# kakaobrain/hqtransformer

Measured on AMD Instinct MI355X. Metric: images/sec (256x256 class-cond sampling), higher is better.
Workload: dtype bf16

## Files before the change

hqtransformer_amd/csrc/engine.hip:

```cpp
#include "../../include/hqt.h"
#include "kernels.h"
#include "fast_kernels.h"
#include "split_kernels.h"
#include "persist.h"

#include <algorithm>
#include <cmath>
#include <cstdarg>
#include <cstdio>
#include <cstring>
#include <map>
#include <memory>
#include <mutex>
#include <string>
#include <vector>

static thread_local std::string g_err;
static int fail(int code, const char* fmt, ...) {
    char buf[1024];
    va_list ap;
    va_start(ap, fmt);
    vsnprintf(buf, sizeof(buf), fmt, ap);
    va_end(ap);
    g_err = buf;
// ... 8 lines not shown
#define CHK(expr)                  \
    do {                           \
        int r_ = (expr);           \
        if (r_ != HQT_OK) return r_; \
    } while (0)

struct DeviceGuard {
    int prev = -1;
    bool ok = false;
    explicit DeviceGuard(int dev) {
        if (hipGetDevice(&prev) != hipSuccess) prev = -1;
        ok = prev == dev || hipSetDevice(dev) == hipSuccess;
        if (prev == dev) prev = -1;
    }
    ~DeviceGuard() { if (prev >= 0) hipSetDevice(prev); }
};
#define ON_DEVICE(h_)                                                                          \
    DeviceGuard dg_((h_)->device);                                                             \
    if (!dg_.ok) return fail(HQT_ERR_HIP, "hipSetDevice(%d) failed", (h_)->device)

struct Tensor {
    float* d = nullptr;
    std::vector<int64_t> shape;
    size_t n = 0;
};

struct Lin {
    const float* w32 = nullptr;
    const float* b32 = nullptr;
    bf16_t* w16 = nullptr;
    half_t* w16h = nullptr;
    half_t* w16l = nullptr;
    float* w32t = nullptr;
    half_t* wfrag16 = nullptr;
    half_t* wup16 = nullptr;
    bf16_t* wpk = nullptr;
    bf16_t* wpk_ln = nullptr;
    float* colsum = nullptr;
    float* bias_ln = nullptr;
    int N = 0, K = 0;
};

struct BlockW {
    bool body = false;
    const float *ln1_g, *ln1_b, *ln2_g, *ln2_b;
    Lin qkv, proj, fc1, fc2;
};

struct DecLayer {
    int kind;
    std::string name;
    int cin, cout, res;
    Lin conv1, conv2, nin, q, k, v, proj;
    const float *n1_g = nullptr, *n1_b = nullptr, *n2_g = nullptr, *n2_b = nullptr;
};

struct PersistProg {
    std::vector<PersistPhase> phases;
    char* stream = nullptr;
    unsigned long long* d_cu_off = nullptr;
    PersistPhase* d_phases = nullptr;
    bool ok = false;
};

struct TimingSlot {
    std::string name;
    std::vector<std::pair<hipEvent_t, hipEvent_t>> ev;
    size_t used = 0;
    int64_t launches = 0;
    double total_ms = 0.0;
};

struct hqt_handle {
    hqt_config cfg;
    int device = 0;
    bool finalized = false;
    std::map<std::string, Tensor> w;
    std::vector<void*> owned;
    size_t workspace_bytes = 0;
    int64_t params[3] = {0, 0, 0};
    std::vector<BlockW> body, depth;
    Lin head_top, head_bot;
    int Tmax = 0;
    int max_prefix = 0;
    static constexpr int BODY_BUFS = 10;
    size_t body_bytes[BODY_BUFS] = {};
    int depth_rows = 0;
    int score_chunk = 0;
    int depth_cap() const { return std::max(cfg.max_batch, score_chunk); }
    static constexpr int DEPTH_BUFS = 4;
    size_t depth_bytes[DEPTH_BUFS] = {};
    float *x = nullptr, *xd = nullptr, *logits = nullptr;
    void *hbuf = nullptr, *qbuf = nullptr, *abuf = nullptr, *mbuf = nullptr;
    void *kcache = nullptr, *vcache = nullptr, *dk = nullptr, *dv = nullptr;
    bf16_t *xpk = nullptr, *xdpk = nullptr;
    float *parts = nullptr, *partsd = nullptr;
    int nparts = 0, npartsd = 0;
    float* fold_tmp = nullptr;
    bool tile_gemm = true;
    float* splitk = nullptr;
    size_t splitk_elems = 0;
    struct { const float* slabs; int S; int rows; const float* bias; } pend = {nullptr, 0, 0, nullptr};
    StepState* state = nullptr;
    RowKey* rows = nullptr;
    static constexpr int ROWS_RING = 4;
    RowKey* rows_pinned[ROWS_RING] = {nullptr, nullptr, nullptr, nullptr};
// ... 573 lines not shown
    CHK(get_w(h, p + ".attn.value.weight", {D, D}, &wv));
    CHK(get_w(h, p + ".attn.query.bias", {D}, &bq));
    CHK(get_w(h, p + ".attn.key.bias", {D}, &bk));
    CHK(get_w(h, p + ".attn.value.bias", {D}, &bv));
    float *wqkv, *bqkv;
    CHK(dev_alloc(h, (void**)&wqkv, (size_t)3 * D * D * 4, false));
    CHK(dev_alloc(h, (void**)&bqkv, (size_t)3 * D * 4, false));
    HIPCHK(hipMemcpy(wqkv, wq, D * D * 4, hipMemcpyDeviceToDevice));
    HIPCHK(hipMemcpy(wqkv + D * D, wk, D * D * 4, hipMemcpyDeviceToDevice));
    HIPCHK(hipMemcpy(wqkv + 2 * D * D, wv, D * D * 4, hipMemcpyDeviceToDevice));
    HIPCHK(hipMemcpy(bqkv, bq, D * 4, hipMemcpyDeviceToDevice));
    HIPCHK(hipMemcpy(bqkv + D, bk, D * 4, hipMemcpyDeviceToDevice));
    HIPCHK(hipMemcpy(bqkv + 2 * D, bv, D * 4, hipMemcpyDeviceToDevice));
    CHK(make_lin(h, b.qkv, wqkv, bqkv, 3 * D, D, true, true));
    CHK(get_w(h, p + ".attn.proj.weight", {D, D}, &w));
    CHK(get_w(h, p + ".attn.proj.bias", {D}, &bias));
    CHK(make_lin(h, b.proj, w, bias, D, D, true, true));
    CHK(get_w(h, p + ".mlp.0.weight", {4 * D, D}, &w));
    CHK(get_w(h, p + ".mlp.0.bias", {4 * D}, &bias));
    CHK(make_lin(h, b.fc1, w, bias, 4 * D, D, true, true));
    CHK(get_w(h, p + ".mlp.2.weight", {D, 4 * D}, &w));
    CHK(get_w(h, p + ".mlp.2.bias", {D}, &bias));
    CHK(make_lin(h, b.fc2, w, bias, D, 4 * D, true, true));
    CHK(fold_ln(h, b.qkv, b.ln1_g, b.ln1_b));
    CHK(fold_ln(h, b.fc1, b.ln2_g, b.ln2_b));
    return HQT_OK;
}

static int load_conv(hqt_handle* h, const std::string& name, int O, int I, int ksz, Lin& l, bool upsampling = false) {
    const float *w, *b;
    CHK(get_w(h, "stage1." + name + ".weight", {O, I, ksz, ksz}, &w));
    CHK(get_w(h, "stage1." + name + ".bias", {O}, &b));
    const int taps = ksz * ksz;
    float* wt = const_cast<float*>(w);
    if (taps > 1) {
        CHK(dev_alloc(h, (void**)&wt, (size_t)O * I * taps * 4, false));
        HIPCHK(launch_repack_conv(w, wt, O, I, taps, 0));
    }
    CHK(make_lin(h, l, wt, b, O, I * taps, false, true));
    if (taps == 9 && I % 32 == 0) {
        if (O % 128 == 0 || O <= 16) {
            CHK(dev_alloc(h, (void**)&l.wfrag16, split_frag_elems(O, I) * sizeof(half_t), false));
            HIPCHK(launch_pack_split_frag16(wt, l.wfrag16, O, I, 0));
        }
        if (upsampling && O % 128 == 0 && I % 64 == 0) {
            CHK(dev_alloc(h, (void**)&l.wup16, split_up_elems(O, I) * sizeof(half_t), false));
            HIPCHK(hipMemset(l.wup16, 0, split_up_elems(O, I) * sizeof(half_t)));
            HIPCHK(launch_pack_split_up16(wt, l.wup16, O, I, 0));
        }
    }
    return HQT_OK;
}

static int conv_in_cpad(const hqt_config& c) { return c.s1_use_init_downsample ? 4 : 16; }

static int load_encoder(hqt_handle* h) {
    const hqt_config& c = h->cfg;
    for (auto& l : h->enc) {
        if (l.kind == 6) {
            const int ks = c.s1_use_init_downsample ? 4 : 3, taps = ks * ks, cp = conv_in_cpad(c);
            const float *w, *b;
            CHK(get_w(h, "stage1.encoder.conv_in.weight", {l.cout, 3, ks, ks}, &w));
            CHK(get_w(h, "stage1.encoder.conv_in.bias", {l.cout}, &b));
            float* wt;
            CHK(dev_alloc(h, (void**)&wt, (size_t)l.cout * cp * taps * 4, false));
            HIPCHK(launch_repack_conv(w, wt, l.cout, 3, taps, 0, cp));
            CHK(make_lin(h, l.conv1, wt, b, l.cout, cp * taps, false));
        } else if (l.kind == 5) {
            CHK(load_conv(h, l.name, l.cout, l.cin, 3, l.conv1));
        } else if (l.kind == 1) {
            CHK(get_w(h, "stage1." + l.name + ".norm1.weight", {l.cin}, &l.n1_g));
            CHK(get_w(h, "stage1." + l.name + ".norm1.bias", {l.cin}, &l.n1_b));
            CHK(get_w(h, "stage1." + l.name + ".norm2.weight", {l.cout}, &l.n2_g));
            CHK(get_w(h, "stage1." + l.name + ".norm2.bias", {l.cout}, &l.n2_b));
            CHK(load_conv(h, l.name + ".conv1", l.cout, l.cin, 3, l.conv1));
            CHK(load_conv(h, l.name + ".conv2", l.cout, l.cout, 3, l.conv2));
            if (l.cin != l.cout) CHK(load_conv(h, l.name + ".nin_shortcut", l.cout, l.cin, 1, l.nin));
        } else if (l.kind == 2) {
            CHK(get_w(h, "stage1." + l.name + ".norm.weight", {l.cin}, &l.n1_g));
            CHK(get_w(h, "stage1." + l.name + ".norm.bias", {l.cin}, &l.n1_b));
            CHK(load_conv(h, l.name + ".q", l.cin, l.cin, 1, l.q));
            CHK(load_conv(h, l.name + ".k", l.cin, l.cin, 1, l.k));
            CHK(load_conv(h, l.name + ".v", l.cin, l.cin, 1, l.v));
            CHK(load_conv(h, l.name + ".proj_out", l.cin, l.cin, 1, l.proj));
        } else {
            CHK(get_w(h, "stage1.encoder.norm_out.weight", {l.cin}, &l.n1_g));
            CHK(get_w(h, "stage1.encoder.norm_out.bias", {l.cin}, &l.n1_b));
            CHK(load_conv(h, "encoder.conv_out", l.cout, l.cin, 3, l.conv1));
        }
    }
    const int E = c.s1_embed_dim, L = c.code_levels == 3 ? 3 : 2;
    CHK(load_conv(h, "quant_conv_b", E, c.s1_z_channels, 1, h->quant_conv));
    if (c.s1_resample == HQT_RESAMPLE_CONV2) {
        const float *w, *b;
        CHK(get_w(h, "stage1.down_t.weight", {E, E, 2, 2}, &w));
        CHK(get_w(h, "stage1.down_t.bias", {E}, &b));
        h->down_lin = Lin();
        h->down_lin.w32 = w; h->down_lin.b32 = b; h->down_lin.N = E; h->down_lin.K = 4 * E;
    }
    for (int l = 0; l < L; ++l) {
        const int dim = c.s1_resample ? E : E << (2 * (L - 1 - l));
        const std::string name = L == 3 ? "stage1.quantizers." + std::to_string(l) + ".embedding"
                                        : (l == 0 ? "stage1.quantize_t.embedding" : "stage1.quantize_b.embedding");
        const float* e = h->w[name].d;
        CHK(dev_alloc(h, (void**)&h->cb_norm[l], (size_t)c.s1_n_embed * 4, false));
        HIPCHK(launch_row_sumsq(e, DT_F32, h->cb_norm[l], c.s1_n_embed, dim, 0));
    }
    h->has_encoder = true;
    return alloc_encode_workspace(h);
}

static std::string key2(const hqt_handle* h, const char* name);

static int finalize_impl(hqt_handle* h);
static int persist_build(hqt_handle* h);
extern "C" int hqt_finalize_weights(hqt_handle* h) {
    if (!h) return fail(HQT_ERR_INVALID, "null handle");
    if (h->finalized) return HQT_OK;
    DeviceGuard dg(h->device);
    if (!dg.ok) return fail(HQT_ERR_HIP, "hipSetDevice(%d) failed", h->device);
    const size_t owned_before = h->owned.size();
    const int rc = finalize_impl(h);
    if (h->fold_tmp) { hipFree(h->fold_tmp); h->fold_tmp = nullptr; }
    if (rc != HQT_OK) {
        hipDeviceSynchronize();
        for (size_t i = owned_before; i < h->owned.size(); ++i) hipFree(h->owned[i]);
        h->owned.resize(owned_before);
        h->body.clear(); h->depth.clear();
        h->pbody = PersistProg(); h->pfull = PersistProg();
        h->head_top = h->head_bot = h->head_l2 = h->post_quant = h->quant_conv = Lin();
        for (auto& l : h->dec) { l.conv1 = l.conv2 = l.nin = l.q = l.k = l.v = l.proj = Lin(); }
        for (auto& l : h->enc) { l.conv1 = l.conv2 = l.nin = l.q = l.k = l.v = l.proj = Lin(); }
        for (auto& p : h->cb_norm) p = nullptr;
        h->vq_h = h->vq_recon = h->vq_zz = h->vq_err = nullptr; h->vq_z = nullptr; h->vq_best = nullptr;
        h->vq_t = h->vq_q = nullptr; h->up_table = nullptr; h->up_lin = h->down_lin = Lin();
        h->has_encoder = false;
    }
// ... 51 lines not shown
            }
            HIPCHK(hipDeviceSynchronize());
        }
        CHK(persist_build(h));
        if (c.cond_type == HQT_COND_CLASS) CHK(get_w(h, "stage2.sos.weight", {c.n_classes, D}, &t));
        else if (c.cond_type == HQT_COND_TEXT) {
            CHK(get_w(h, "stage2.tok_emb_txt.weight", {c.vocab_txt, D}, &t));
            CHK(get_w(h, "stage2.pos_emb_txt.weight", {c.ctx_len_txt, D}, &t));
        } else CHK(get_w(h, "stage2.sos", {1, 1, D}, &t));
    }
    if (c.has_stage1) {
        const int E = c.s1_embed_dim;
        const float* t;
        if (c.code_levels == 3) {
            CHK(get_w(h, "stage1.quantizers.0.embedding", {c.s1_n_embed, 16 * E}, &t));
            CHK(get_w(h, "stage1.quantizers.1.embedding", {c.s1_n_embed, 4 * E}, &t));
            CHK(get_w(h, "stage1.quantizers.2.embedding", {c.s1_n_embed, E}, &t));
            CHK(load_conv(h, "post_quant_conv_b", c.s1_z_channels, E, 1, h->post_quant));
        } else {
            CHK(get_w(h, "stage1.quantize_t.embedding", {c.s1_n_embed, c.s1_resample ? E : 4 * E}, &t));
            if (c.s1_resample == HQT_RESAMPLE_CONV2) {
                const float *uw, *ub;
                CHK(get_w(h, "stage1.upsample_t.weight", {E, E, 2, 2}, &uw));
                CHK(get_w(h, "stage1.upsample_t.bias", {E}, &ub));
                CHK(dev_alloc(h, (void**)&h->up_table, (size_t)c.s1_n_embed * 4 * E * 4, false));
                HIPCHK(launch_fold_upsample_t(t, uw, ub, h->up_table, c.s1_n_embed, E, 0));
                float *wt, *b4;
                CHK(dev_alloc(h, (void**)&wt, (size_t)4 * E * E * 4, false));
                CHK(dev_alloc(h, (void**)&b4, (size_t)4 * E * 4, false));
                HIPCHK(launch_repack_upsample_t(uw, ub, wt, b4, E, 0));
                h->up_lin = Lin();
                h->up_lin.w32 = wt; h->up_lin.b32 = b4; h->up_lin.N = 4 * E; h->up_lin.K = E;
            }
            CHK(get_w(h, "stage1.quantize_b.embedding", {c.s1_n_embed, E}, &t));
            CHK(load_conv(h, "post_quant_conv_b", c.s1_z_channels, 2 * E, 1, h->post_quant));
        }
        for (auto& l : h->dec) {
            if (l.kind == 0 || l.kind == 3) CHK(load_conv(h, l.name, l.cout, l.cin, 3, l.conv1, l.kind == 3));
            else if (l.kind == 1) {
                CHK(get_w(h, "stage1." + l.name + ".norm1.weight", {l.cin}, &l.n1_g));
                CHK(get_w(h, "stage1." + l.name + ".norm1.bias", {l.cin}, &l.n1_b));
                CHK(get_w(h, "stage1." + l.name + ".norm2.weight", {l.cout}, &l.n2_g));
                CHK(get_w(h, "stage1." + l.name + ".norm2.bias", {l.cout}, &l.n2_b));
                CHK(load_conv(h, l.name + ".conv1", l.cout, l.cin, 3, l.conv1));
                CHK(load_conv(h, l.name + ".conv2", l.cout, l.cout, 3, l.conv2));
                if (l.cin != l.cout) CHK(load_conv(h, l.name + ".nin_shortcut", l.cout, l.cin, 1, l.nin));
            } else if (l.kind == 2) {
                CHK(get_w(h, "stage1." + l.name + ".norm.weight", {l.cin}, &l.n1_g));
                CHK(get_w(h, "stage1." + l.name + ".norm.bias", {l.cin}, &l.n1_b));
                CHK(load_conv(h, l.name + ".q", l.cin, l.cin, 1, l.q));
                CHK(load_conv(h, l.name + ".k", l.cin, l.cin, 1, l.k));
                CHK(load_conv(h, l.name + ".v", l.cin, l.cin, 1, l.v));
                CHK(load_conv(h, l.name + ".proj_out", l.cin, l.cin, 1, l.proj));
            } else {
                CHK(get_w(h, "stage1.decoder.norm_out.weight", {l.cin}, &l.n1_g));
                CHK(get_w(h, "stage1.decoder.norm_out.bias", {l.cin}, &l.n1_b));
                CHK(load_conv(h, "decoder.conv_out", l.cout, l.cin, 3, l.conv1));
            }
        }
    }
    if (c.has_stage1 && h->w.count("stage1.encoder.conv_in.weight") && (c.s1_resample != HQT_RESAMPLE_CONV2 || h->w.count("stage1.down_t.weight")))
        CHK(load_encoder(h));
    HIPCHK(stream_gemm_configure());
    HIPCHK(tile_gemm_configure());
    HIPCHK(mfma_gemm_configure());
    HIPCHK(split_kernels_configure());
    HIPCHK(hipDeviceSynchronize());
    h->finalized = true;
    return HQT_OK;
}

struct Mode {
    bool fast = false;
    bool split = false;
    bool split_ar = false;
    int act_dt() const { return fast ? DT_BF16 : DT_F32; }
    size_t act_sz() const { return fast ? 2 : 4; }
};
static int mode_of(int precision, bool stage1, Mode* md) {
    if (precision == HQT_PRECISION_FAST) md->fast = true;
    else if (precision == HQT_PRECISION_SPLIT && stage1) md->split = true;
    else if (precision == HQT_PRECISION_SPLIT) md->split_ar = true;
    else if (precision != HQT_PRECISION_EXACT) return fail(HQT_ERR_INVALID, "unknown precision %d", precision);
    return HQT_OK;
}

static void lin_args(const hqt_handle* h, GemmArgs& g, const Lin& l, bool split_planes) {
    g.N = l.N; g.K = l.K; g.ldb = l.K;
    g.bias = l.b32;
    g.zero_page = h->zero_page;
    g.tune = h->policy;
    if (g.alpha == 0.0f) g.alpha = 1.0f;
    if (g.lda == 0) g.lda = l.K;
    if (split_planes) { g.Bw = l.w16h; g.Bw_lo = l.w16l; g.Bw_frag16 = l.wfrag16; g.Bw_up16 = l.wup16; }
}

struct SlotName {
    char s[64];
    SlotName(const char* tag, int rows) {
        static const bool by_rows = getenv("HQT_TIMING_BY_ROWS") != nullptr;
        snprintf(s, sizeof s, by_rows ? "%s@%d" : "%s", tag, rows);
    }
};

static int ar_linear(hqt_handle* h, const Mode& md, GemmArgs g, const Lin& l, int a_dt, int c_dt, hipStream_t st,
                     const char* tag, bool defer_residual = false, int* resid_nparts = nullptr) {
// ... 1276 lines not shown
    hqt_handle* h = c.h;
    hipStream_t st = c.st;
    const int adt = c.adt, n = c.n;
    void *&cur = c.cur, *&t1 = c.t1, *&t2 = c.t2;
    const int res = l.res, hw = res * res;
    if (l.kind == 0 || l.kind == 3) {
        const int ro = l.kind == 3 ? 2 * res : res;
        GemmArgs g = conv_args(cur, n, ro, l.cin, 9, l.kind == 3, t1, l.cout);
        S1Operand a = S1_PLANES;
        if (c.cur_planes) c.cur_planes = false;
        else CHK(s1_plain(c, &g, l.conv1, &a));
        CHK(s1_conv(c, g, a, l.conv1, adt, "conv3x3"));
        std::swap(cur, t1);
    } else if (l.kind == 5) {
        GemmArgs g = conv_args(cur, n, res / 2, l.cin, 9, 0, t1, l.cout);
        g.conv_stride2 = 1; g.conv_nopad = 1;
        CHK(s1_conv(c, g, S1_TENSOR, l.conv1, adt, "conv_down"));
        std::swap(cur, t1);
    } else if (l.kind == 1) {
        GemmArgs g = conv_args(cur, n, res, l.cin, 9, 0, t1, l.cout);
        S1Operand a;
        CHK(s1_norm(c, cur, l.cin, hw, c.gn1, l.n1_g, l.n1_b, 1, &g, l.conv1, &a));
        CHK(s1_conv(c, g, a, l.conv1, adt, "conv3x3"));
        const void* shortcut = cur;
        void* outbuf = t2;
        if (l.cin != l.cout) {
            GemmArgs sc = conv_args(cur, n, res, l.cin, 1, 0, t2, l.cout);
            CHK(s1_plain(c, &sc, l.nin, &a));
            CHK(s1_conv(c, sc, a, l.nin, adt, "conv1x1"));
            shortcut = t2;
            outbuf = cur;
        }
        g = conv_args(t1, n, res, l.cout, 9, 0, outbuf, l.cout);
        g.resid = shortcut;
        CHK(s1_norm(c, t1, l.cout, hw, c.gn2, l.n2_g, l.n2_b, 1, &g, l.conv2, &a));
        bool planes = false;
        if (a == S1_PLANES && next && next->kind == 3 && next->cin == l.cout) {
            GemmArgs up = conv_args(outbuf, n, 2 * res, next->cin, 9, 1, t1, next->cout);
            GemmArgs me = g;
            lin_args(h, me, l.conv2, true);
            planes = split_shape_ok(h, up, next->conv1) && split_conv3_emits_planes(me);
        }
        if (planes) { g.out_split = 1; g.range_flag = h->range_flag; }
        CHK(s1_conv(c, g, a, l.conv2, adt, "conv3x3"));
        if (outbuf == t2) std::swap(cur, t2);
        c.cur_planes = planes;
        if (planes) count_variant(h, "variant:conv3x3_planes_out:conv3x3");
    } else if (l.kind == 2) {
        const int C = l.cin;
        GemmArgs g = conv_args(cur, n, res, C, 1, 0, h->aq, C);
        S1Operand a;
        CHK(s1_norm(c, cur, C, hw, c.gn1, l.n1_g, l.n1_b, 0, &g, l.q, &a));
        const GemmArgs normed = g;
        CHK(s1_conv(c, g, a, l.q, adt, "conv1x1"));
        g = normed; g.C = h->ak;
        CHK(s1_conv(c, g, a, l.k, adt, "conv1x1"));
        g = normed; g.C = h->av;
        g.store = STORE_NCHW; g.rows_per_image = hw;
        CHK(s1_conv(c, g, a, l.v, adt, "conv1x1"));
        auto product = [&](const void* A, const void* B, void* out, int M, int N, int K, float alpha) -> int {
            Timed t(h, "attn_gemm", st);
            GemmArgs sg{};
            sg.A = A; sg.lda = K; sg.a_batch_stride = (long long)M * K;
            sg.Bw = B; sg.ldb = K; sg.b_batch_stride = (long long)N * K;
            sg.C = out; sg.ldc = N; sg.c_batch_stride = (long long)M * N;
            sg.M = M; sg.N = N; sg.K = K; sg.batch = n; sg.alpha = alpha; sg.store = STORE_ROWS;
            sg.zero_page = h->zero_page;
            if (c.md.fast && mfma_gemm_ok(sg, adt, adt, adt)) {
                count_variant(h, "variant:mfma_gemm:attn_gemm");
                HIPCHK(launch_mfma_gemm(sg, adt, adt, adt, st));
            } else if (s1_split_product(h, c.md, sg)) {
                count_variant(h, "variant:split_gemm:attn_gemm");
                HIPCHK(launch_split_gemm(sg, st));
            } else {
                count_variant(h, c.md.fast ? "variant:gemm_generic_bf16:attn_gemm" : "variant:gemm_generic_f32:attn_gemm");
                HIPCHK(launch_gemm_generic(sg, adt, adt, adt, st));
            }
            return HQT_OK;
        };
        CHK(product(h->aq, h->ak, h->as, hw, hw, C, 1.0f / sqrtf((float)C)));
        { Timed t(h, "softmax", st); HIPCHK(launch_softmax_rows(h->as, adt, n * hw, hw, st)); }
        CHK(product(h->as, h->av, h->ao, hw, C, hw, 1.0f));
        g = conv_args(h->ao, n, res, C, 1, 0, t1, C);
        g.resid = cur;
        CHK(s1_plain(c, &g, l.proj, &a));
        CHK(s1_conv(c, g, a, l.proj, adt, "conv1x1"));
        std::swap(cur, t1);
    } else {
        return fail(HQT_ERR_INVALID, "s1_layer: kind %d", l.kind);
    }
    return HQT_OK;
}

static int decode_chunk(hqt_handle* h, int n, const int64_t* code_t, const int64_t* code_m, const int64_t* code_b, int seq_layout,
                        float* out, int clamp01, const Mode& md, hipStream_t st) {
    const hqt_config& cf = h->cfg;
    const int adt = md.act_dt();
    const int r = h->dec.front().res, E = cf.s1_embed_dim;
    const bool l3 = cf.code_levels == 3;
    {
        Timed t(h, "quant_gather", st);
        if (l3) {
            QuantArgs3 q{code_t, code_m, code_b, seq_layout, W1(h, "quantizers.0.embedding"), W1(h, "quantizers.1.embedding"),
                         W1(h, "quantizers.2.embedding"), h->quant, n, r, E, adt, cf.s1_n_embed};
            HIPCHK(launch_quant_gather3(q, st));
        } else if (cf.s1_resample) {
            const bool conv2 = cf.s1_resample == HQT_RESAMPLE_CONV2;
            QuantRowsArgs q{code_t, code_b, seq_layout, conv2 ? h->up_table : W1(h, "quantize_t.embedding"), conv2 ? 4 : 1,
                            conv2 ? W1(h, "upsample_t.bias") : nullptr, W1(h, "quantize_b.embedding"), h->quant, n, r, E, adt, cf.s1_n_embed};
            HIPCHK(launch_quant_gather_rows(q, st));
        } else {
            QuantArgs q{code_t, code_b, seq_layout, W1(h, "quantize_t.embedding"), W1(h, "quantize_b.embedding"), h->quant, n, r, E, adt, cf.s1_n_embed};
            HIPCHK(launch_quant_gather(q, st));
        }
    }
    S1Ctx c{h, n, md, st, adt, h->act[0], h->act[1], h->act[2], h->act[3], h->gn, h->gn + (size_t)h->dec_chunk * 64};
    {
        GemmArgs g = conv_args(h->quant, n, r, l3 ? E : 2 * E, 1, 0, c.cur, cf.s1_z_channels);
        S1Operand a;
        CHK(s1_plain(c, &g, h->post_quant, &a));
        CHK(s1_conv(c, g, a, h->post_quant, adt, "conv1x1"));
    }
    for (size_t li = 0; li < h->dec.size(); ++li) {
        const DecLayer& l = h->dec[li];
        if (l.kind != 4) { CHK(s1_layer(c, l, li + 1 < h->dec.size() ? &h->dec[li + 1] : nullptr)); continue; }
        const int hw = l.res * l.res;
        GemmArgs g = conv_args(c.cur, n, l.res, l.cin, 9, 0, out, l.cout);
        g.store = STORE_NCHW; g.rows_per_image = hw; g.clamp01 = clamp01;
        if (md.split && l.conv1.w32) {
            GemmArgs d = g;
            d.N = l.conv1.N; d.K = l.conv1.K; d.Bw = l.conv1.w32; d.bias = l.conv1.b32; d.alpha = 1.0f;
            with_gn(d, c.gn1, l.n1_g, l.n1_b, 1);
            if (conv_out_direct_ok(d)) {
                CHK(s1_split_stats(c, c.cur, l.cin, hw, c.gn1));
                Timed t(h, "conv_out", st);
// ... 243 lines not shown
```

hqtransformer_amd/csrc/split_conv.hip:

```cpp
#include "split_kernels.h"
#include "split_ring.h"
#include "gemm_generic.h"
#include <algorithm>
#include <cstdlib>
#include <type_traits>

namespace {
__device__ __forceinline__ unsigned pack_h2(half_t a, half_t b) {
    return (unsigned)__builtin_bit_cast(unsigned short, a) | ((unsigned)__builtin_bit_cast(unsigned short, b) << 16);
}

__device__ __forceinline__ void xcd_tile(int& tile_m, int& tile_n) {
    const int nx = gridDim.x, total = gridDim.x * gridDim.y;
    int id = blockIdx.x + nx * blockIdx.y;
    if ((total & 7) == 0) id = (id & 7) * (total >> 3) + (id >> 3);
    tile_m = id / nx;
    tile_n = id - tile_m * nx;
}
}

__global__ void split_f32_kernel(const float* __restrict__ src, half_t* __restrict__ hi, half_t* __restrict__ lo, size_t n) {
    for (size_t i = blockIdx.x * (size_t)blockDim.x + threadIdx.x; i < n; i += (size_t)gridDim.x * blockDim.x) split2(src[i], hi[i], lo[i]);
}
hipError_t launch_split_f32(const float* src, half_t* hi, half_t* lo, size_t n, hipStream_t st) {
// ... 625 lines not shown
                } else {
#pragma unroll
                    for (int e = 0; e < 4; ++e)
                        if (n4 + e < g.N) {
                            const long long idx = (long long)m * ldc + n4 + e;
                            float x = apply_act(s[e] * g.alpha + bq[e], act);
                            if (Rb) x += Rb[idx];
                            Cb[idx] = x;
                        }
                }
            }
    }
    }
#ifdef HQT_SPLIT_GEMM_STAMPS
    if (g.am_best && tid == 0) {
        st_[3] = clock64();
        long long* d = reinterpret_cast<long long*>(g.am_best) + (size_t)(blockIdx.x + gridDim.x * (blockIdx.y + gridDim.y * blockIdx.z)) * 4;
        d[0] = st_[1] - st_[0]; d[1] = st_[2] - st_[1]; d[2] = st_[3] - st_[2]; d[3] = wall_clock64();
    }
#endif
}

__global__ __launch_bounds__(256) void split_rows_combine_kernel(float* C, int ldc, const float* resid, const float* __restrict__ slabs,
                                                                 const float* __restrict__ bias, int M, int N, int S, int act) {
    const long long i = (long long)blockIdx.x * 256 + threadIdx.x, n4 = N >> 2;
    if (i >= (long long)M * n4) return;
    const int m = (int)(i / n4), n = (int)(i - (long long)m * n4) * 4;
    f32x4 v = *reinterpret_cast<const f32x4*>(slabs + (size_t)m * N + n);
    for (int z = 1; z < S; ++z) v += *reinterpret_cast<const f32x4*>(slabs + ((size_t)z * M + m) * N + n);
    if (bias) v += *reinterpret_cast<const f32x4*>(bias + n);
    if (act != ACT_NONE)
#pragma unroll
        for (int e = 0; e < 4; ++e) v[e] = apply_act(v[e], act);
    if (resid) v += *reinterpret_cast<const f32x4*>(resid + (long long)m * ldc + n);
    *reinterpret_cast<f32x4*>(C + (long long)m * ldc + n) = v;
}

int split_gemm_slices(const GemmArgs& g) {
    if (!g.a_f32 || g.b_f32 || g.store != STORE_ROWS || g.rows_per_group != 0 || g.batch > 1 || g.conv_taps) return 1;
    if (g.N % 4 != 0 || g.ldc % 4 != 0 || g.alpha != 1.0f) return 1;
    const int tiles = ((g.N + 127) / 128) * ((g.M + 127) / 128);
    int S = 1;
    while (S < 4 && g.K % (S * 2 * 64) == 0 && (tiles * S * 2 <= 256 || (tiles * S * 2 <= 512 && g.K / (S * 2) >= 1536))) S *= 2;
    return S;
}

bool split_gemm_ok(const GemmArgs& g) {
    if (!g.zero_page || (!g.Bw_lo && !g.b_f32) || g.gn_stats || g.a_packed_mb || g.a_rows_per_group) return false;
    if (g.conv_taps > 1 || g.conv_stride2 || g.upsample) return false;
    if (g.K % 64 != 0 || g.ldb % 8 != 0) return false;
    if (g.a_f32 && (g.conv_taps ? g.Cin : g.lda) % 4 != 0) return false;
    if (g.b_f32 && (!g.a_f32 || g.ldb % 4 != 0)) return false;
    if (g.store == STORE_QKV)
        return g.a_f32 && !g.b_f32 && g.qkv_D > 0 && g.qkv_D % 64 == 0 && g.N % 64 == 0 && g.ldc % 4 == 0 && g.rows_per_group > 0 && !g.resid && !g.qkv_v_pk && g.batch <= 1;
    if (g.store != STORE_ROWS && g.store != STORE_NCHW) return false;
    if (g.store == STORE_ROWS && g.rows_per_group != 0) return false;
    if (g.store == STORE_NCHW && (g.resid || g.act != ACT_NONE)) return false;
    return true;
}
hipError_t launch_split_gemm(const GemmArgs& g0, hipStream_t st) {
    GemmArgs g = g0;
    if (g.conv_taps == 1) { g.lda = g.a_f32 ? g.Cin : 2 * g.Cin; g.conv_taps = 0; }
    const int a_lo_off = g.lda / 2;
    if (g.k_slices > 1 && (!g.k_slabs || g.k_slices > split_gemm_slices(g))) g.k_slices = 1;
    const int S = g.k_slices > 1 ? g.k_slices : 1;
    const dim3 grid((g.N + 127) / 128, (g.M + 127) / 128, S > 1 ? S : (g.batch > 0 ? g.batch : 1));
    if (g.a_f32 && g.b_f32) split_gemm_kernel<true, true><<<grid, 256, 2 * 4 * 128 * 64, st>>>(g, a_lo_off);
    else if (g.a_f32) split_gemm_kernel<true, false><<<grid, 256, 2 * 4 * 128 * 64, st>>>(g, a_lo_off);
    else split_gemm_kernel<false, false><<<grid, 256, 2 * 4 * 128 * 64, st>>>(g, a_lo_off);
    if (S > 1) {
        const long long n = (long long)g.M * (g.N / 4);
        split_rows_combine_kernel<<<(unsigned)((n + 255) / 256), 256, 0, st>>>(reinterpret_cast<float*>(g.C), g.ldc, reinterpret_cast<const float*>(g.resid), g.k_slabs, g.bias, g.M, g.N, S, g.act);
    }
    return hipGetLastError();
}

hipError_t split_kernels_configure() {
    hipError_t e = split_stream_configure();
    if (e != hipSuccess) return e;
    e = hipFuncSetAttribute(reinterpret_cast<const void*>(conv3x3_split_kernel<false, 128, 1>), hipFuncAttributeMaxDynamicSharedMemorySize, split_conv3_lds(128));
    if (e != hipSuccess) return e;
    e = hipFuncSetAttribute(reinterpret_cast<const void*>(conv3x3_split_kernel<true, 32, 1>), hipFuncAttributeMaxDynamicSharedMemorySize, split_conv3_lds(32));
    if (e != hipSuccess) return e;
    e = hipFuncSetAttribute(reinterpret_cast<const void*>(split_gemm_kernel<true, true>), hipFuncAttributeMaxDynamicSharedMemorySize, 2 * 4 * 128 * 64);
    if (e != hipSuccess) return e;
    e = hipFuncSetAttribute(reinterpret_cast<const void*>(split_gemm_kernel<true, false>), hipFuncAttributeMaxDynamicSharedMemorySize, 2 * 4 * 128 * 64);
    if (e != hipSuccess) return e;
    return hipFuncSetAttribute(reinterpret_cast<const void*>(split_gemm_kernel<false, false>), hipFuncAttributeMaxDynamicSharedMemorySize, 2 * 4 * 128 * 64);
}
```

hqtransformer_amd/csrc/split_kernels.h:

```cpp
#pragma once
#include "common.h"
#include "kernels.h"

typedef _Float16 half_t;

hipError_t launch_split_f32(const float* src, half_t* hi, half_t* lo, size_t n, hipStream_t st);

hipError_t launch_split_pack(const float* x, half_t* y, const float* stats, const float* gamma, const float* beta, int B, int HW,
                             int C, int groups, int swish, int* range_flag, hipStream_t st);

bool split_conv3_ok(const GemmArgs& g);
bool split_gemm_ok(const GemmArgs& g);
hipError_t launch_split_conv3(const GemmArgs& g, hipStream_t st);
hipError_t launch_split_gemm(const GemmArgs& g, hipStream_t st);
int split_gemm_slices(const GemmArgs& g);
int split_conv3_tiles_per_image(const GemmArgs& g);
hipError_t split_kernels_configure();

size_t split_frag_elems(int N, int Cin);
hipError_t launch_pack_split_frag16(const float* w_tapmajor, half_t* out, int N, int Cin, hipStream_t st);
size_t split_up_elems(int N, int Cin);
hipError_t launch_pack_split_up16(const float* w_tapmajor, half_t* out, int N, int Cin, hipStream_t st);
bool split_stream_ok(const GemmArgs& g);
bool split_conv3_emits_planes(const GemmArgs& g);
int split_stream_tiles_per_image(const GemmArgs& g);
hipError_t launch_split_conv3_stream(const GemmArgs& g, hipStream_t st);
hipError_t split_stream_configure();
bool conv_out_direct_ok(const GemmArgs& g);
hipError_t launch_conv_out_direct(const GemmArgs& g, hipStream_t st);
```

Baseline: 1700.

## Fuse stage-1 attention QKV projection and add single-kernel split-fp16 attention

Concatenates the q/k/v 1x1 conv weights into one fused projection so a single split GEMM writes Q, K and V. It then replaces the separate score product, softmax and value product with one kernel per 64-query block that keeps scores in LDS and uses hi/lo fp16 MFMA. This removes several launches and the round trips of the score matrix through global memory in the VQ-GAN attention blocks. It adds extra weight memory, is limited to hw<=256 with C%128==0, and relaxes the QKV-store check to allow non-f32 A operands.

```diff
diff --git a/hqtransformer_amd/csrc/engine.hip b/hqtransformer_amd/csrc/engine.hip
--- a/hqtransformer_amd/csrc/engine.hip
+++ b/hqtransformer_amd/csrc/engine.hip
@@ -84,6 +84,7 @@
     std::string name;
     int cin, cout, res;
     Lin conv1, conv2, nin, q, k, v, proj;
+    Lin qkv;
     const float *n1_g = nullptr, *n1_b = nullptr, *n2_g = nullptr, *n2_b = nullptr;
 };
 
@@ -763,6 +764,25 @@
     return HQT_OK;
 }
 
+static int fuse_qkv(hqt_handle* h, DecLayer& l) {
+    l.qkv = Lin();
+    if (!l.q.w16h || !l.k.w16h || !l.v.w16h) return HQT_OK;
+    const size_t C = (size_t)l.cin, e = C * C;
+    const Lin* part[3] = {&l.q, &l.k, &l.v};
+    half_t *wh, *wl;
+    float* b;
+    CHK(dev_alloc(h, (void**)&wh, 3 * e * sizeof(half_t), false));
+    CHK(dev_alloc(h, (void**)&wl, 3 * e * sizeof(half_t), false));
+    CHK(dev_alloc(h, (void**)&b, 3 * C * sizeof(float), false));
+    for (int i = 0; i < 3; ++i) {
+        HIPCHK(hipMemcpy(wh + i * e, part[i]->w16h, e * sizeof(half_t), hipMemcpyDeviceToDevice));
+        HIPCHK(hipMemcpy(wl + i * e, part[i]->w16l, e * sizeof(half_t), hipMemcpyDeviceToDevice));
+        HIPCHK(hipMemcpy(b + i * C, part[i]->b32, C * sizeof(float), hipMemcpyDeviceToDevice));
+    }
+    l.qkv.w16h = wh; l.qkv.w16l = wl; l.qkv.b32 = b; l.qkv.N = (int)(3 * C); l.qkv.K = (int)C;
+    return HQT_OK;
+}
+
 static int conv_in_cpad(const hqt_config& c) { return c.s1_use_init_downsample ? 4 : 16; }
 
 static int load_encoder(hqt_handle* h) {
@@ -794,6 +814,7 @@
             CHK(load_conv(h, l.name + ".k", l.cin, l.cin, 1, l.k));
             CHK(load_conv(h, l.name + ".v", l.cin, l.cin, 1, l.v));
             CHK(load_conv(h, l.name + ".proj_out", l.cin, l.cin, 1, l.proj));
+            CHK(fuse_qkv(h, l));
         } else {
             CHK(get_w(h, "stage1.encoder.norm_out.weight", {l.cin}, &l.n1_g));
             CHK(get_w(h, "stage1.encoder.norm_out.bias", {l.cin}, &l.n1_b));
@@ -951,6 +972,7 @@
                 CHK(load_conv(h, l.name + ".k", l.cin, l.cin, 1, l.k));
                 CHK(load_conv(h, l.name + ".v", l.cin, l.cin, 1, l.v));
                 CHK(load_conv(h, l.name + ".proj_out", l.cin, l.cin, 1, l.proj));
+                CHK(fuse_qkv(h, l));
             } else {
                 CHK(get_w(h, "stage1.decoder.norm_out.weight", {l.cin}, &l.n1_g));
                 CHK(get_w(h, "stage1.decoder.norm_out.bias", {l.cin}, &l.n1_b));
@@ -2333,6 +2355,31 @@
         S1Operand a;
         CHK(s1_norm(c, cur, C, hw, c.gn1, l.n1_g, l.n1_b, 0, &g, l.q, &a));
         const GemmArgs normed = g;
+        GemmArgs f = normed;
+        bool fused = false;
+        if (a == S1_PLANES && l.qkv.w16h && split_attn_ok(C, hw)) {
+            const char* e = getenv("HQT_ATTN_FUSED");
+            lin_args(h, f, l.qkv, true);
+            f.store = STORE_QKV; f.C = h->aq; f.C2 = h->ak; f.C3 = h->av; f.qkv_D = C; f.qkv_first = 0;
+            f.rows_per_group = f.M; f.group_stride = f.M;
+            fused = !(e && atoi(e) == 0) && split_gemm_ok(f);
+        }
+        if (fused) {
+            {
+                Timed t(h, SlotName("conv1x1", f.M).s, st);
+                for (int i = 0; i < 3; ++i) count_variant(h, "variant:split_gemm:conv1x1");
+                count_variant(h, "fused:split_gemm_qkv:conv1x1");
+                HIPCHK(launch_split_gemm(f, st));
+            }
+            {
+                Timed t(h, "attn_gemm", st);
+                for (int i = 0; i < 2; ++i) count_variant(h, "variant:split_gemm:attn_gemm");
+                count_variant(h, "fused:split_attn:attn_gemm");
+                const SplitAttnArgs sa{reinterpret_cast<const float*>(h->aq), reinterpret_cast<const float*>(h->ak), reinterpret_cast<const float*>(h->av),
+                                       reinterpret_cast<float*>(h->ao), n, hw, C, 1.0f / sqrtf((float)C), h->range_flag, nullptr};
+                HIPCHK(launch_split_attn(sa, st));
+            }
+        } else {
         CHK(s1_conv(c, g, a, l.q, adt, "conv1x1"));
         g = normed; g.C = h->ak;
         CHK(s1_conv(c, g, a, l.k, adt, "conv1x1"));
@@ -2362,6 +2409,7 @@
         CHK(product(h->aq, h->ak, h->as, hw, hw, C, 1.0f / sqrtf((float)C)));
         { Timed t(h, "softmax", st); HIPCHK(launch_softmax_rows(h->as, adt, n * hw, hw, st)); }
         CHK(product(h->as, h->av, h->ao, hw, C, hw, 1.0f));
+        }
         g = conv_args(h->ao, n, res, C, 1, 0, t1, C);
         g.resid = cur;
         CHK(s1_plain(c, &g, l.proj, &a));
diff --git a/hqtransformer_amd/csrc/split_conv.hip b/hqtransformer_amd/csrc/split_conv.hip
--- a/hqtransformer_amd/csrc/split_conv.hip
+++ b/hqtransformer_amd/csrc/split_conv.hip
@@ -701,7 +701,7 @@
     if (g.a_f32 && (g.conv_taps ? g.Cin : g.lda) % 4 != 0) return false;
     if (g.b_f32 && (!g.a_f32 || g.ldb % 4 != 0)) return false;
     if (g.store == STORE_QKV)
-        return g.a_f32 && !g.b_f32 && g.qkv_D > 0 && g.qkv_D % 64 == 0 && g.N % 64 == 0 && g.ldc % 4 == 0 && g.rows_per_group > 0 && !g.resid && !g.qkv_v_pk && g.batch <= 1;
+        return !g.b_f32 && g.qkv_D > 0 && g.qkv_D % 64 == 0 && g.N % 64 == 0 && g.ldc % 4 == 0 && g.rows_per_group > 0 && !g.resid && !g.qkv_v_pk && g.batch <= 1;
     if (g.store != STORE_ROWS && g.store != STORE_NCHW) return false;
     if (g.store == STORE_ROWS && g.rows_per_group != 0) return false;
     if (g.store == STORE_NCHW && (g.resid || g.act != ACT_NONE)) return false;
@@ -724,8 +724,336 @@
     return hipGetLastError();
 }
 
+namespace {
+constexpr int AT_QB = 64;
+constexpr int AT_KEYS = 256;
+constexpr int AT_SPITCH = AT_KEYS * 4 + 16;
+constexpr int AT_S_BYTES = AT_QB * AT_SPITCH;
+constexpr int AT_STAGE = 2 * (AT_QB + AT_KEYS) * 64;
+constexpr int AT_VPLANE = 16 * 256 * 4;
+constexpr int AT_LDS = AT_S_BYTES + 2 * AT_STAGE;
+static_assert(2 * AT_VPLANE <= AT_STAGE, "the v pair images fit a stage");
+static_assert(AT_LDS <= 160 * 1024, "LDS budget");
+}
+
+__global__ __launch_bounds__(256, 1) void split_attn_kernel(SplitAttnArgs a) {
+    extern __shared__ __attribute__((aligned(16))) char lds_raw[];
+    char* const Sb = lds_raw;
+    char* const stage0 = lds_raw + AT_S_BYTES;
+    const int tid = threadIdx.x, lane = tid & 63, wave = tid >> 6, fr = lane & 31, fh = lane >> 5;
+    const int HW = a.hw, C = a.C;
+    const int nqb = HW / AT_QB, nwg = gridDim.x;
+    int wg = blockIdx.x;
+    if ((nwg & 7) == 0) wg = (wg & 7) * (nwg >> 3) + (wg >> 3);
+    const int img = wg / nqb, q0 = (wg - img * nqb) * AT_QB;
+    const float* const Q = a.q + ((long long)img * HW + q0) * C;
+    const float* const K = a.k + (long long)img * HW * C;
+    const float* const V = a.v + (long long)img * HW * C;
+    float* const O = a.o + ((long long)img * HW + q0) * C;
+    bool bad = false;
+    f32x16 accm[2][2], accx[2][2];
+    auto clear = [&]() {
+#pragma unroll
+        for (int i = 0; i < 2; ++i)
+#pragma unroll
+            for (int j = 0; j < 2; ++j)
+#pragma unroll
+                for (int r = 0; r < 16; ++r) { accm[i][j][r] = 0.0f; accx[i][j][r] = 0.0f; }
+    };
+    auto mfma3 = [&](const half8 (&ah)[2], const half8 (&al)[2], const half8 (&wh)[2], const half8 (&wl)[2]) {
+#pragma unroll
+        for (int i = 0; i < 2; ++i)
+#pragma unroll
+            for (int j = 0; j < 2; ++j) {
+                accm[i][j] = __builtin_amdgcn_mfma_f32_32x32x16_f16(wh[j], ah[i], accm[i][j], 0, 0, 0);
+                accx[i][j] = __builtin_amdgcn_mfma_f32_32x32x16_f16(wh[j], al[i], accx[i][j], 0, 0, 0);
+            }
+#pragma unroll
+        for (int i = 0; i < 2; ++i)
+#pragma unroll
+            for (int j = 0; j < 2; ++j) accx[i][j] = __builtin_amdgcn_mfma_f32_32x32x16_f16(wl[j], ah[i], accx[i][j], 0, 0, 0);
+    };
+    auto split_piece = [&](const u32x4& x0, const u32x4& x1, u32x4& hi4, u32x4& lo4) {
+        float xs[8];
+#pragma unroll
+        for (int e = 0; e < 4; ++e) {
+            const unsigned b0 = x0[e], b1 = x1[e];
+            xs[e] = __builtin_bit_cast(float, b0);
+            xs[4 + e] = __builtin_bit_cast(float, b1);
+        }
+        unsigned hi[4], lo[4];
+        split8_checked(xs, hi, lo, bad);
+        hi4 = u32x4{hi[0], hi[1], hi[2], hi[3]};
+        lo4 = u32x4{lo[0], lo[1], lo[2], lo[3]};
+    };
+
+    const int prow = tid >> 2, pch = ((tid & 3) ^ ((prow >> 2) & 3)) * 8;
+    const u32x4 zero4 = {0u, 0u, 0u, 0u};
+    u32x4 sl0[5][2], sl1[5][2];
+    auto fetch1 = [&](int kt, u32x4 (&sl)[5][2]) {
+        const int k0 = kt * 32 + pch;
+        const float* s = Q + (long long)prow * C + k0;
+        sl[0][0] = *reinterpret_cast<const u32x4*>(s);
+        sl[0][1] = *reinterpret_cast<const u32x4*>(s + 4);
+#pragma unroll
+        for (int it = 0; it < 4; ++it) {
+            const int row = it * 64 + prow;
+            const float* sk = K + (long long)min(row, HW - 1) * C + k0;
+            sl[1 + it][0] = *reinterpret_cast<const u32x4*>(sk);
+            sl[1 + it][1] = *reinterpret_cast<const u32x4*>(sk + 4);
+        }
+    };
+    auto convert1 = [&](u32x4 (&sl)[5][2]) {
+#pragma unroll
+        for (int p = 0; p < 5; ++p) {
+            const bool ok = p == 0 || (p - 1) * 64 + prow < HW;
+            const u32x4 x0 = ok ? sl[p][0] : zero4, x1 = ok ? sl[p][1] : zero4;
+            split_piece(x0, x1, sl[p][0], sl[p][1]);
+        }
+    };
+    auto write1 = [&](int buf, const u32x4 (&cv)[5][2]) {
+        char* const st = stage0 + (size_t)buf * AT_STAGE;
+#pragma unroll
+        for (int p = 0; p < 5; ++p) {
+            char* const at = p == 0 ? st + tid * 16 : st + 2 * AT_QB * 64 + (p - 1) * 4096 + tid * 16;
+            *reinterpret_cast<u32x4*>(at) = cv[p][0];
+            *reinterpret_cast<u32x4*>(at + (p == 0 ? AT_QB * 64 : AT_KEYS * 64)) = cv[p][1];
+        }
+    };
+    const bool keys_mine = wave * 64 < HW;
+    auto compute1 = [&](int buf) {
+        const char* const Ah = stage0 + (size_t)buf * AT_STAGE, *Al = Ah + AT_QB * 64, *Wh = Ah + 2 * AT_QB * 64, *Wl = Wh + AT_KEYS * 64;
+#pragma unroll
+        for (int ks = 0; ks < 2; ++ks) {
+            const int c = ks * 2 + fh;
+            half8 ah[2], al[2], wh[2], wl[2];
+#pragma unroll
+            for (int i = 0; i < 2; ++i) {
+                const int r = i * 32 + fr;
+                const int o = r * 64 + ((c ^ ((r >> 2) & 3)) << 4);
+                ah[i] = *reinterpret_cast<const half8*>(Ah + o);
+                al[i] = *reinterpret_cast<const half8*>(Al + o);
+            }
+#pragma unroll
+            for (int j = 0; j < 2; ++j) {
+                const int r = wave * 64 + j * 32 + fr;
+                const int o = r * 64 + ((c ^ ((r >> 2) & 3)) << 4);
+                wh[j] = *reinterpret_cast<const half8*>(Wh + o);
+                wl[j] = *reinterpret_cast<const half8*>(Wl + o);
+            }
+            mfma3(ah, al, wh, wl);
+        }
+    };
+#ifdef HQT_SPLIT_ATTN_STAMPS
+    long long st_[5];
+    st_[0] = clock64();
+#endif
+    clear();
+    const int KT1 = C / 32;
+    auto step1 = [&](int kt, int buf, u32x4 (&into)[5][2], u32x4 (&conv)[5][2]) {
+        fetch1(min(kt + 2, KT1 - 1), into);
+        __builtin_amdgcn_sched_barrier(0);
+        compute1(buf);
+        convert1(conv);
+        __builtin_amdgcn_sched_barrier(0);
+        write1(buf ^ 1, conv);
+        __syncthreads();
+    };
+    fetch1(0, sl0);
+    fetch1(1, sl1);
+    convert1(sl0);
+    write1(0, sl0);
+    __syncthreads();
+    for (int kt = 0; kt < KT1; kt += 2) {
+        step1(kt, 0, sl0, sl1);
+        step1(kt + 1, 1, sl1, sl0);
+    }
+#ifdef HQT_SPLIT_ATTN_STAMPS
+    st_[1] = clock64();
+#endif
+    if (keys_mine) {
+#pragma unroll
+        for (int i = 0; i < 2; ++i)
+#pragma unroll
+            for (int j = 0; j < 2; ++j)
+#pragma unroll
+                for (int q4 = 0; q4 < 4; ++q4) {
+                    f32x4 v;
+#pragma unroll
+                    for (int e = 0; e < 4; ++e) v[e] = (accm[i][j][4 * q4 + e] + accx[i][j][4 * q4 + e] * SPLIT_INV) * a.alpha + 0.0f;
+                    *reinterpret_cast<f32x4*>(Sb + (i * 32 + fr) * AT_SPITCH + (wave * 64 + j * 32 + 8 * q4 + 4 * fh) * 4) = v;
+                }
+    }
+    __syncthreads();
+
+    const int KT2 = HW / 32, T = ((C + 255) / 256) * KT2;
+    const int cq = tid & 63;
+    u32x4 vl0[4][2], vl1[4][2];
+    auto fetch2 = [&](int t, u32x4 (&vl)[4][2]) {
+        const int nc = t / KT2, kt = t - nc * KT2;
+        const int c = nc * 256 + cq * 4;
+        const bool ok = c < C;
+#pragma unroll
+        for (int it = 0; it < 4; ++it) {
+            const int j = kt * 32 + (it * 4 + wave) * 2;
+            const float* sv = V + (long long)j * C + (ok ? c : 0);
+            vl[it][0] = *reinterpret_cast<const u32x4*>(sv);
+            vl[it][1] = *reinterpret_cast<const u32x4*>(sv + C);
+        }
+    };
+    auto convert2 = [&](int t, u32x4 (&vl)[4][2]) {
+        const bool ok = (min(t, T - 1) / KT2) * 256 + cq * 4 < C;
+#pragma unroll
+        for (int it = 0; it < 4; ++it) {
+            const u32x4 k0 = ok ? vl[it][0] : zero4, k1 = ok ? vl[it][1] : zero4;
+            const u32x4 x0 = {k0[0], k1[0], k0[1], k1[1]}, x1 = {k0[2], k1[2], k0[3], k1[3]};
+            split_piece(x0, x1, vl[it][0], vl[it][1]);
+        }
+    };
+    auto write2 = [&](int buf, const u32x4 (&cv)[4][2]) {
+        char* const st = stage0 + (size_t)buf * AT_STAGE;
+#pragma unroll
+        for (int it = 0; it < 4; ++it) {
+            char* const at = st + (it * 4 + wave) * 1024 + cq * 16;
+            *reinterpret_cast<u32x4*>(at) = cv[it][0];
+            *reinterpret_cast<u32x4*>(at + AT_VPLANE) = cv[it][1];
+        }
+    };
+    auto compute2 = [&](int buf, int kt) {
+        const char* const Vh = stage0 + (size_t)buf * AT_STAGE, *Vl = Vh + AT_VPLANE;
+#pragma unroll
+        for (int ks = 0; ks < 2; ++ks) {
+            half8 ah[2], al[2], wh[2], wl[2];
+#pragma unroll
+            for (int i = 0; i < 2; ++i) {
+                const int o = (i * 32 + fr) * AT_SPITCH + (kt * 32 + ks * 16 + fh * 8) * 2;
+                ah[i] = *reinterpret_cast<const half8*>(Sb + o);
+                al[i] = *reinterpret_cast<const half8*>(Sb + o + AT_KEYS * 2);
+            }
+#pragma unroll
+            for (int j = 0; j < 2; ++j) {
+                const int o = (ks * 8 + fh * 4) * 1024 + (wave * 64 + j * 32 + fr) * 4;
+                u32x4 uh, ul;
+#pragma unroll
+                for (int w = 0; w < 4; ++w) {
+                    uh[w] = *reinterpret_cast<const unsigned*>(Vh + o + w * 1024);
+                    ul[w] = *reinterpret_cast<const unsigned*>(Vl + o + w * 1024);
+                }
+                wh[j] = __builtin_bit_cast(half8, uh);
+                wl[j] = __builtin_bit_cast(half8, ul);
+            }
+            mfma3(ah, al, wh, wl);
+        }
+    };
+#ifdef HQT_SPLIT_ATTN_STAMPS
+    st_[2] = clock64();
+#endif
+    fetch2(0, vl0);
+    fetch2(1, vl1);
+    __builtin_amdgcn_sched_barrier(0);
+
+    {
+        float* const rmax = reinterpret_cast<float*>(stage0), *rsum = rmax + 4 * AT_QB;
+        const int nseg = HW >> 6;
+        const bool seg_mine = wave < nseg;
+        char* const row = Sb + lane * AT_SPITCH;
+        float x[64];
+        if (seg_mine) {
+            float m = -INFINITY;
+#pragma unroll
+            for (int i = 0; i < 16; ++i) {
+                const f32x4 v = *reinterpret_cast<const f32x4*>(row + wave * 256 + i * 16);
+#pragma unroll
+                for (int e = 0; e < 4; ++e) { x[4 * i + e] = v[e]; m = fmaxf(m, v[e]); }
+            }
+            rmax[wave * AT_QB + lane] = m;
+        }
+        __syncthreads();
+        if (seg_mine) {
+            float m = rmax[lane];
+            for (int s = 1; s < nseg; ++s) m = fmaxf(m, rmax[s * AT_QB + lane]);
+            float t[32];
+#pragma unroll
+            for (int i = 0; i < 64; ++i) x[i] = expf(x[i] - m);
+#pragma unroll
+            for (int i = 0; i < 32; ++i) t[i] = x[i] + x[i + 32];
+#pragma unroll
+            for (int w = 16; w > 0; w >>= 1)
+#pragma unroll
+                for (int i = 0; i < w; ++i) t[i] = t[i] + t[i + w];
+            rsum[wave * AT_QB + lane] = t[0];
+        }
+        __syncthreads();
+        if (seg_mine) {
+            float tot = rsum[lane];
+            for (int s = 1; s < nseg; ++s) tot = tot + rsum[s * AT_QB + lane];
+#pragma unroll
+            for (int i = 0; i < 8; ++i) {
+                float ps[8];
+#pragma unroll
+                for (int e = 0; e < 8; ++e) ps[e] = x[8 * i + e] / tot;
+                unsigned hi[4], lo[4];
+                split8_checked(ps, hi, lo, bad);
+                *reinterpret_cast<u32x4*>(row + wave * 128 + i * 16) = u32x4{hi[0], hi[1], hi[2], hi[3]};
+                *reinterpret_cast<u32x4*>(row + AT_KEYS * 2 + wave * 128 + i * 16) = u32x4{lo[0], lo[1], lo[2], lo[3]};
+            }
+        }
+    }
+    __syncthreads();
+
+#ifdef HQT_SPLIT_ATTN_STAMPS
+    st_[3] = clock64();
+#endif
+    convert2(0, vl0);
+    write2(0, vl0);
+    __syncthreads();
+    auto step2 = [&](int t, int buf, u32x4 (&into)[4][2], u32x4 (&conv)[4][2]) {
+        const int nc = t / KT2, kt = t - nc * KT2;
+        if (kt == 0) clear();
+        fetch2(min(t + 2, T - 1), into);
+        __builtin_amdgcn_sched_barrier(0);
+        compute2(buf, kt);
+        convert2(t + 1, conv);
+        __builtin_amdgcn_sched_barrier(0);
+        write2(buf ^ 1, conv);
+        __syncthreads();
+        if (kt == KT2 - 1 && nc * 256 + wave * 64 < C) {
+#pragma unroll
+            for (int i = 0; i < 2; ++i)
+#pragma unroll
+                for (int j = 0; j < 2; ++j)
+#pragma unroll
+                    for (int q4 = 0; q4 < 4; ++q4) {
+                        f32x4 v;
+#pragma unroll
+                        for (int e = 0; e < 4; ++e) v[e] = (accm[i][j][4 * q4 + e] + accx[i][j][4 * q4 + e] * SPLIT_INV) * 1.0f + 0.0f;
+                        *reinterpret_cast<f32x4*>(O + (long long)(i * 32 + fr) * C + nc * 256 + wave * 64 + j * 32 + 8 * q4 + 4 * fh) = v;
+                    }
+        }
+    };
+    for (int t = 0; t < T; t += 2) {
+        step2(t, 0, vl0, vl1);
+        step2(t + 1, 1, vl1, vl0);
+    }
+    if (bad && a.range_flag) atomicOr(a.range_flag, 1);
+#ifdef HQT_SPLIT_ATTN_STAMPS
+    if (a.stamps && tid == 0) {
+        st_[4] = clock64();
+        for (int i = 0; i < 4; ++i) a.stamps[(size_t)blockIdx.x * 4 + i] = st_[i + 1] - st_[i];
+    }
+#endif
+}
+
+bool split_attn_ok(int C, int hw) { return C > 0 && C % 128 == 0 && hw >= AT_QB && hw <= AT_KEYS && hw % AT_QB == 0; }
+hipError_t launch_split_attn(const SplitAttnArgs& a, hipStream_t st) {
+    split_attn_kernel<<<dim3(a.hw / AT_QB * a.n, 1, 1), 256, AT_LDS, st>>>(a);
+    return hipGetLastError();
+}
+
 hipError_t split_kernels_configure() {
     hipError_t e = split_stream_configure();
+    if (e != hipSuccess) return e;
+    e = hipFuncSetAttribute(reinterpret_cast<const void*>(split_attn_kernel), hipFuncAttributeMaxDynamicSharedMemorySize, AT_LDS);
     if (e != hipSuccess) return e;
     e = hipFuncSetAttribute(reinterpret_cast<const void*>(conv3x3_split_kernel<false, 128, 1>), hipFuncAttributeMaxDynamicSharedMemorySize, split_conv3_lds(128));
     if (e != hipSuccess) return e;
diff --git a/hqtransformer_amd/csrc/split_kernels.h b/hqtransformer_amd/csrc/split_kernels.h
--- a/hqtransformer_amd/csrc/split_kernels.h
+++ b/hqtransformer_amd/csrc/split_kernels.h
@@ -13,6 +13,16 @@
 bool split_gemm_ok(const GemmArgs& g);
 hipError_t launch_split_conv3(const GemmArgs& g, hipStream_t st);
 hipError_t launch_split_gemm(const GemmArgs& g, hipStream_t st);
+struct SplitAttnArgs {
+    const float *q, *k, *v;
+    float* o;
+    int n, hw, C;
+    float alpha;
+    int* range_flag;
+    long long* stamps;
+};
+bool split_attn_ok(int C, int hw);
+hipError_t launch_split_attn(const SplitAttnArgs& a, hipStream_t st);
 int split_gemm_slices(const GemmArgs& g);
 int split_conv3_tiles_per_image(const GemmArgs& g);
 hipError_t split_kernels_configure();
```

Result: no change. 1715 (median of 6 runs) (+0.9%).
